# Autobot37/weatherforecastingtoolkit

Measured on AMD Instinct MI355X. Metric: SEVIR 384x384 frames/sec (AE train step), higher is better.
Workload: dtype f32; 1 GPU; experiments/ae_v2 conv AE (ae_64x8x8_lin.PosAwareAE_TF, img_size=384), 1x384x384 synthetic SEVIR frames, batch 32/GPU, fp32, fwd + L1 + bwd + AdamW + cosine-warmup LR; batch_per_gpu=32, global_batch=32, img_size=384, parallelism=dp1, params=215033281

## Files before the change

### include/wfae.h

```cpp
#ifndef WFAE_H
#define WFAE_H

#include <stddef.h>
#include <stdint.h>

#ifdef __cplusplus
extern "C" {
#endif

typedef void* wfae_stream_t;

typedef enum {
  WFAE_OK = 0,
  WFAE_ERR_BAD_SHAPE = -1,
  WFAE_ERR_NULL_POINTER = -2,
  WFAE_ERR_WORKSPACE = -3,
  WFAE_ERR_LAUNCH = -4,
  WFAE_ERR_UNSUPPORTED = -5
} wfae_status;

int wfae_version(void);
const char* wfae_last_error_string(void);
size_t wfae_workspace_bytes(int64_t max_weight_elems);

enum { WFAE_PRECISION_FP32 = 0, WFAE_PRECISION_BF16 = 1 };
int wfae_set_matmul_precision(int mode);
int wfae_get_matmul_precision(void);

int wfae_set_split_gemm(int on);
int wfae_get_split_gemm(void);

int wfae_set_c1n(int on);
int wfae_get_c1n(void);

int wfae_conv1x1_fwd(const float* x, const float* w, const float* bias, const float* res,
                     int64_t res_img_stride, float* y, int NB, int Cin, int Cout, int HW,
                     wfae_stream_t stream);
int wfae_conv1x1_fwd_stats(const float* x, const float* w, const float* bias, const float* res,
                           int64_t res_img_stride, float* y, int NB, int Cin, int Cout, int HW,
                           double* stat_part, int64_t stat_capacity, int* stat_rows, wfae_stream_t stream);
int wfae_conv1x1_fwd_bnact(const float* x, const float* bn_scale, const float* bn_shift, const float* w,
                           const float* bias, const float* res, int64_t res_img_stride, float* y, int NB, int Cin,
                           int Cout, int HW, double* stat_part, int64_t stat_capacity, int* stat_rows,
                           wfae_stream_t stream);
int wfae_conv1x1_bwd_weight_bnact(const float* dy, const float* x, const float* bn_scale, const float* bn_shift,
                                  float* dw, int NB, int Cin, int Cout, int HW, int accumulate, void* ws,
                                  size_t ws_bytes, wfae_stream_t stream);
int wfae_conv1x1_bwd_data(const float* dy, const float* w, float* dx, int NB, int Cin, int Cout,
                          int HW, wfae_stream_t stream);
int wfae_conv1x1_bwd_weight(const float* dy, const float* x, float* dw, int NB, int Cin, int Cout,
                            int HW, int accumulate, void* ws, size_t ws_bytes, wfae_stream_t stream);

int wfae_c1r_supported(int M, int K, int HW);
int wfae_c1r_stat_rows(int M, int K, int NB, int HW);
int wfae_c1r_fwd(const float* w, int64_t w_sm, int64_t w_sk, const float* x, const float* pro_scale, const float* pro_shift,
                 const float* res, float* y, int NB, int K, int M, int HW, double* stat_part, int64_t stat_capacity,
                 int* stat_rows, wfae_stream_t stream);
int wfae_c1r_bnred_supported(int M, int K, int HW);
int wfae_c1r_bnred(const float* w, int64_t w_sm, int64_t w_sk, const float* dt, const float* x, const float* bn_scale,
                   const float* bn_shift, const float* save_mean, const float* save_invstd, float* da, int NB, int K, int M, int HW,
                   double* part, int64_t part_capacity, int* part_rows, wfae_stream_t stream);
int wfae_bn_act_bwd_from_rows(const double* part, int rows, int C, float* dgamma, float* dbeta, int accumulate, void* ws,
                              size_t ws_bytes, wfae_stream_t stream);
int wfae_c1r_bndx(const float* w, int64_t w_sm, int64_t w_sk, const float* dt, const float* x, const float* gamma,
                  const float* bn_scale, const float* bn_shift, const float* save_mean, const float* save_invstd, const float* coef,
                  const float* res, float* dx, int NB, int K, int M, int HW, int training, wfae_stream_t stream);
int wfae_c1rb_supported(int M, int K, int HW);
int wfae_c1rb_stat_rows(int M, int K, int NB, int HW);
int wfae_c1rb_fwd(const float* w, int64_t w_sm, int64_t w_sk, const uint16_t* x, const float* pro_scale, const float* pro_shift,
                  const uint16_t* res, uint16_t* y, int NB, int K, int M, int HW, double* stat_part, int64_t stat_capacity,
                  int* stat_rows, wfae_stream_t stream);
int wfae_c1w_supported(int Cin, int Cout, int HW);
int wfae_c1w_bwd_weight(const float* dy, const float* x, const float* bn_scale, const float* bn_shift, float* dw, int NB, int Cin,
                        int Cout, int HW, int accumulate, void* ws, size_t ws_bytes, wfae_stream_t stream);
int wfae_c1w_bwd_weight_bf16(const uint16_t* dy, const uint16_t* x, const float* bn_scale, const float* bn_shift, float* dw, int NB,
                             int Cin, int Cout, int HW, int accumulate, void* ws, size_t ws_bytes, wfae_stream_t stream);
int wfae_set_c1wd(int on);
int wfae_get_c1wd(void);
int wfae_c1wd_supported(int C, int mid, int HW);
int wfae_c1wd_bwd(const float* dy, const float* t2, const float* bn_scale, const float* bn_shift, const float* w3, float* dw3,
                  float* da3, int NB, int C, int mid, int HW, int accumulate, void* ws, size_t ws_bytes, wfae_stream_t stream);
int wfae_linear_fwd(const float* x, const float* w, const float* bias, float* y, int B, int In,
                    int Out, void* ws, size_t ws_bytes, wfae_stream_t stream);
int wfae_linear_bwd_data(const float* dy, const float* w, float* dx, int B, int In, int Out,
                         wfae_stream_t stream);
int wfae_linear_bwd_weight(const float* dy, const float* x, float* dw, int B, int In, int Out,
                           int accumulate, wfae_stream_t stream);
int wfae_linear_bwd_data_splitk(const float* dy, const float* w, float* dx, int B, int In, int Out, void* ws,
                                size_t ws_bytes, wfae_stream_t stream);
int wfae_linear_bwd_weight_splitk(const float* dy, const float* x, float* dw, int B, int In, int Out, int accumulate,
                                  void* ws, size_t ws_bytes, wfae_stream_t stream);

int wfae_conv4x4s2_down(const float* hi, const float* w, float* lo, int NB, int Chi, int Clo,
                        int Hlo, int Wlo, wfae_stream_t stream);
int wfae_conv4x4s2_up(const float* lo, const float* w, float* hi, int NB, int Chi, int Clo, int Hlo,
                      int Wlo, void* ws, size_t ws_bytes, wfae_stream_t stream);
int wfae_conv4x4s2_wgrad(const float* lo, const float* hi, float* dw, int NB, int Chi, int Clo,
                         int Hlo, int Wlo, int accumulate, void* ws, size_t ws_bytes,
                         wfae_stream_t stream);

int wfae_dconv_fwd(const float* x, const float* w, const float* bias, float* y, int NB, int Cin,
                   int Cout, int H, int W, int KS, int stride, int pad, int groups,
                   wfae_stream_t stream);
int wfae_dconv_bwd_data(const float* dy, const float* w, float* dx, int NB, int Cin, int Cout,
                        int H, int W, int KS, int pad, int groups, wfae_stream_t stream);
int wfae_dconv_bwd_weight(const float* dy, const float* x, float* dw, int NB, int Cin, int Cout,
                          int H, int W, int KS, int stride, int pad, int groups, int accumulate,
                          void* ws, size_t ws_bytes, wfae_stream_t stream);

int wfae_gconv3x3_fwd(const float* x, const float* w, float* y, int NB, int C, int H, int W, int groups,
                      int transposed, void* ws, size_t ws_bytes, wfae_stream_t stream);
int wfae_gconv3x3_bwd_weight(const float* dy, const float* x, float* dw, int NB, int C, int H, int W,
                             int groups, int accumulate, void* ws, size_t ws_bytes, wfae_stream_t stream);

int wfae_bn_stats_train(const float* x, int NB, int C, int HW, const float* gamma,
                        const float* beta, float eps, float momentum, float* running_mean,
                        float* running_var, float* save_mean, float* save_invstd, float* scale,
                        float* shift, void* ws, size_t ws_bytes, wfae_stream_t stream);
int wfae_bn_stats_from_rows(const double* stat_part, int rows, int NB, int C, int HW, const float* gamma,
                            const float* beta, float eps, float momentum, float* running_mean,
                            float* running_var, float* save_mean, float* save_invstd, float* scale,
                            float* shift, void* ws, size_t ws_bytes, wfae_stream_t stream);
int wfae_bn_fold_eval(const float* gamma, const float* beta, const float* running_mean,
                      const float* running_var, float eps, float* save_mean, float* save_invstd,
                      float* scale, float* shift, int C, wfae_stream_t stream);
int wfae_bn_act_fwd(const float* x, const float* scale, const float* shift, float* y, int NB, int C,
                    int HW, int act, wfae_stream_t stream);
int wfae_bn_act_fwd_stats(const float* x, const float* scale, const float* shift, float* y, int NB, int C, int HW, int act,
                          double* part, int64_t part_capacity, int* splits_out, wfae_stream_t stream);
int wfae_bn_stats_from_parts(const double* part, int splits, int NB, int C, int HW, const float* gamma, const float* beta,
                             float eps, float momentum, float* running_mean, float* running_var, float* save_mean,
                             float* save_invstd, float* scale, float* shift, wfae_stream_t stream);
int wfae_bn_act_bwd(const float* dy, const float* x, const float* gamma, const float* scale,
                    const float* shift, const float* save_mean, const float* save_invstd,
                    const float* res, float* dx, float* dgamma, float* dbeta, int NB, int C, int HW,
                    int act, int training, int accumulate, int phases, void* ws, size_t ws_bytes,
                    wfae_stream_t stream);

int wfae_convert_f32_to_bf16(const float* src, uint16_t* dst, int64_t n, wfae_stream_t stream);
int wfae_convert_bf16_to_f32(const uint16_t* src, float* dst, int64_t n, wfae_stream_t stream);
int wfae_bn_stats_train_bf16(const uint16_t* x, int NB, int C, int HW, const float* gamma, const float* beta, float eps,
                             float momentum, float* running_mean, float* running_var, float* save_mean, float* save_invstd,
                             float* scale, float* shift, void* ws, size_t ws_bytes, wfae_stream_t stream);
int wfae_bn_act_fwd_bf16(const uint16_t* x, const float* scale, const float* shift, uint16_t* y, int NB, int C, int HW, int act,
                         wfae_stream_t stream);
int wfae_bn_act_fwd_stats_bf16(const uint16_t* x, const float* scale, const float* shift, uint16_t* y, int NB, int C, int HW,
                               int act, double* part, int64_t part_capacity, int* splits_out, wfae_stream_t stream);
int wfae_conv1x1_fwd_bf16(const uint16_t* x, const float* bn_scale, const float* bn_shift, const float* w, const float* bias,
                          const uint16_t* res, int64_t res_img_stride, uint16_t* y, int NB, int Cin, int Cout, int HW,
                          double* stat_part, int64_t stat_capacity, int* stat_rows, wfae_stream_t stream);
int wfae_conv1x1_bwd_data_bf16(const uint16_t* dy, const float* w, uint16_t* dx, int NB, int Cin, int Cout, int HW,
                               wfae_stream_t stream);
int wfae_conv1x1_bwd_weight_bf16(const uint16_t* dy, const uint16_t* x, const float* bn_scale, const float* bn_shift, float* dw,
                                 int NB, int Cin, int Cout, int HW, int accumulate, void* ws, size_t ws_bytes,
                                 wfae_stream_t stream);
int wfae_gconv3x3_fwd_bf16(const uint16_t* x, const float* w, uint16_t* y, int NB, int C, int H, int W, int groups,
                           int transposed, void* ws, size_t ws_bytes, wfae_stream_t stream);
int wfae_gconv3x3_bwd_weight_bf16(const uint16_t* dy, const uint16_t* x, float* dw, int NB, int C, int H, int W, int groups,
                                  int accumulate, void* ws, size_t ws_bytes, wfae_stream_t stream);
int wfae_dconv_fwd_bf16out(const float* x, const float* w, const float* bias, uint16_t* y, int NB, int Cout, int H, int W,
                           wfae_stream_t stream);
int wfae_dconv_fwd_bf16in(const uint16_t* x, const float* w, const float* bias, float* y, int NB, int Cin, int Cout, int H,
                          int W, wfae_stream_t stream);
int wfae_dconv_bwd_data_bf16out(const float* dy, const float* w, uint16_t* dx, int NB, int Cin, int H, int W,
// ... 316 lines not shown
```

### weatherforecastingtoolkit_amd/functional.py

```python
from __future__ import annotations

import os

import torch
from torch.autograd import Function

from . import ops

BN_EPS = 1e-5


_overlap = False
_side = {}


STAT_FUSION = os.environ.get("WFAE_STAT_FUSION", "1") == "1"


FUSE_A1 = os.environ.get("WFAE_FUSE_A1", "1") == "1"
FUSE_A1_MAXC = 1 << 30
FUSE_A3 = os.environ.get("WFAE_FUSE_A3", "1") == "1"
FUSE_A3_MAXC = int(os.environ.get("WFAE_FUSE_A3_MAXC", "128"))
FUSE_A3_MAXC_C1R = max(FUSE_A3_MAXC, 256)

# ... 374 lines not shown
        (x,) = ctx.saved_tensors
        return ops.leaky_relu_bwd(_c(dy), x)


class MeanFn(Function):

    @staticmethod
    def forward(ctx, x, hinge, sign, weight):
        x = _c(x)
        ctx.save_for_backward(x)
        ctx.cfg = (hinge, sign, weight)
        return ops.mean_fwd(x, hinge, sign, weight)

    @staticmethod
    def backward(ctx, g):
        (x,) = ctx.saved_tensors
        hinge, sign, weight = ctx.cfg
        return ops.mean_bwd(x, _c(g), hinge, sign, weight), None, None, None


class ScaleByFn(Function):

    @staticmethod
    def forward(ctx, x, s):
        ctx.save_for_backward(s)
        return ops.scale(_c(x), 1.0, s)

    @staticmethod
    def backward(ctx, g):
        (s,) = ctx.saved_tensors
        return ops.scale(_c(g), 1.0, s), None


def hinge_d_loss(logits_real, logits_fake):
    return AddFn.apply(MeanFn.apply(logits_real, True, -1.0, 0.5), MeanFn.apply(logits_fake, True, 1.0, 0.5))


def neg_mean(x):
    return MeanFn.apply(x, False, 1.0, -1.0)


def _g3_fwd(x, w, groups):
    if ops.gconv3x3_supported(x.shape[1], groups) and w.shape[0] == x.shape[1]:
        return ops.gconv3x3_fwd(x, w, groups, False)
    return ops.dconv_fwd(x, w, None, 3, 1, 1, groups)


def _g3_dgrad(dy, w, cin, groups):
    if ops.gconv3x3_supported(cin, groups) and w.shape[0] == cin:
        return ops.gconv3x3_fwd(dy, w, groups, True)
    return ops.dconv_bwd_data(dy, w, cin, 3, 1, groups)


def _g3_wgrad(dy, x, dw, groups):
    c = x.shape[1]
    if c % groups == 0 and c // groups in (4, 8, 16, 32) and dw.shape[0] == c and groups > 1:
        return ops.gconv3x3_bwd_weight(dy, x, dw, groups)
    return ops.dconv_bwd_weight(dy, x, dw, 3, 1, 1, groups)


def _mk_stats(mean, invstd, scale, shift):
    st = ops.BnStats.__new__(ops.BnStats)
    st.mean, st.invstd, st.scale, st.shift = mean, invstd, scale, shift
    return st


def _storage(t):
    return "bf16" if t.dtype == ops.BF16 else "f32"


def _c1(w, plane, transposed, x, st=None, res=None, stats=False, fam=None):
    if fam is None:
        fam = ops.conv1x1_route("dgrad" if transposed else "fwd", w.shape[1] if transposed else w.shape[0], x.shape[1],
                                x.shape[2] * x.shape[3], _storage(x), st is not None, False, "none" if res is None else "ordinary")
    if fam == "c1b" and (plane is None or plane.numel() == 0):
        fam = "gemm"
    label = None if fam in ("c1r", "gemm") else "wfae_c1b_dgrad" if transposed else "wfae_c1b_fwd"
    return ops._c1_launch(fam, plane if fam == "c1b" else w, transposed, x, st, None, res, False, stats, label)


_b16 = _c1


def _dgrad_bn(dt, w, Wt, x, gamma, st, dgamma, dbeta, res, training):
    how = ops.conv1x1_dgrad_bn_route(w.shape[1], dt.shape[1], dt.shape[2] * dt.shape[3], _storage(dt))
    if how is not None:
        da, sr = ops.c1r_bnred(w, dt, x, st, store=how == "bnred")
        ops.bn_act_bwd_from_rows(sr, x.shape[1], dgamma, dbeta)
        if how == "bndx":
            return ops.c1r_bndx(w, dt, x, gamma, st, res, training)
        return ops.bn_act_bwd_dx(da, x, gamma, st, res, 1, training)
    return ops.bn_act_bwd(_c1(w, Wt, True, dt)[0], x, gamma, st, dgamma, dbeta, res, 1, training)


class BottleneckFn(Function):
    @staticmethod
    def forward(ctx, x, g1, b1, w1, g2, b2, wg, g3, b3, w3, mod, x_stats=None):
        xc = _c(x)
        if xc is not x:
            x_stats = None
        x = xc
        bn1, bn2, bn3 = mod.f[0], mod.f[3], mod.f[6]
        groups = mod.f[5].groups
        training = _use_batch_stats(bn1)
        fuse = training and STAT_FUSION
        emit = fuse and getattr(mod, "emit_stats", False)
        C, mid, hw = x.shape[1], w1.shape[0], x.shape[2] * x.shape[3]
        sto = _storage(x)

        def route(op, m, k, pro=False, res="none"):
            return ops.conv1x1_route(op, m, k, hw, sto, pro, False, res)
        fused1 = FUSE_A1 and C <= FUSE_A1_MAXC and ops.conv1x1_bnact_supported(x, mid)
        r1, r3 = route("fwd", mid, C, fused1), route("fwd", C, mid, True, "ordinary")
        fused3 = (FUSE_A3 and C <= (FUSE_A3_MAXC_C1R if r3 in ("c1r", "c1rb") else FUSE_A3_MAXC)
                  and ops.conv1x1_bnact_supported((x.shape[0], mid) + x.shape[2:], C))
        if not fused3:
            r3 = route("fwd", C, mid, False, "ordinary")
        d1, d3 = (route("dgrad", C, mid), route("dgrad", mid, C)) if sto == "bf16" else (None, None)
        W1p, W3p = (ops.c1b_weights(w1), ops.c1b_weights(w3)) if "c1b" in (r1, r3, d1, d3) else ((None, None), (None, None))
        st1 = _bn_stats_rows(x_stats if (fuse or isinstance(x_stats, ops.StatParts)) else None, x, bn1, training)
        a1 = None if fused1 else ops.bn_act_fwd(x, st1, 1)
        t1, sr2 = _c1(w1, W1p[0], False, *((x, st1) if fused1 else (a1, None)), None, fuse, r1)
        st2 = _bn_stats_rows(sr2, t1, bn2, training)
        a2 = ops.bn_act_fwd(t1, st2, 1)
        t2 = _g3_fwd(a2, wg, groups)
        st3 = _bn_stats(t2, bn3, training)
        a3 = None if fused3 else ops.bn_act_fwd(t2, st3, 1)
        y, mod._out_stats = _c1(w3, W3p[0], False, *((t2, st3) if fused3 else (a3, None)), x, emit, r3)
        ctx.save_for_backward(x, _opt(a1), t1, a2, t2, _opt(a3), g1, w1, g2, wg, g3, w3,
                              st1.mean, st1.invstd, st1.scale, st1.shift,
                              st2.mean, st2.invstd, st2.scale, st2.shift,
                              st3.mean, st3.invstd, st3.scale, st3.shift,
                              _opt(W1p[1] if d1 == "c1b" else None), _opt(W3p[1] if d3 == "c1b" else None))
        ctx.training = training
        ctx.groups = groups
        ctx.betas = (b1, b2, b3)
        return y

    @staticmethod
    def backward(ctx, dy):
        (x, a1, t1, a2, t2, a3, g1, w1, g2, wg, g3, w3, *s) = ctx.saved_tensors
        st1, st2, st3 = _mk_stats(*s[0:4]), _mk_stats(*s[4:8]), _mk_stats(*s[8:12])
        W1t, W3t = s[12], s[13]
        tr = ctx.training
        dy = _c(dy)
        mid = w1.shape[0]
        dw3 = grad_buffer(w3)
        da3 = None
        if a3.numel() == 0:
            if ops.conv1x1_wd_route(dy.shape[1], mid, dy.shape[2] * dy.shape[3], _storage(dy)) == "c1wd":
                da3 = _on_main(lambda: ops.conv1x1_bwd_wd(dy, t2, st3, w3, dw3))
            if da3 is None:
                _wgrad(lambda: ops.conv1x1_bwd_weight_bnact(dy, t2, st3, dw3), dy, t2, st3.scale, st3.shift)
        else:
            _wgrad(lambda: ops.conv1x1_bwd_weight(dy, a3, dw3), dy, a3)
        dg3, db3 = grad_buffer(g3), grad_buffer(ctx.betas[2])
        if da3 is not None:
            dt2 = ops.bn_act_bwd(da3, t2, g3, st3, dg3, db3, None, 1, tr)
        else:
            dt2 = _dgrad_bn(dy, w3, W3t, t2, g3, st3, dg3, db3, None, tr)
        del da3
        dwg = grad_buffer(wg)
        _wgrad(lambda: _g3_wgrad(dt2, a2, dwg, ctx.groups), dt2, a2)
        da2 = _g3_dgrad(dt2, wg, mid, ctx.groups)
        del dt2
        dg2, db2 = grad_buffer(g2), grad_buffer(ctx.betas[1])
        dt1 = ops.bn_act_bwd(da2, t1, g2, st2, dg2, db2, None, 1, tr)
        del da2
        dw1 = grad_buffer(w1)
        if a1.numel() == 0:
            _wgrad(lambda: ops.conv1x1_bwd_weight_bnact(dt1, x, st1, dw1), dt1, x, st1.scale, st1.shift)
        else:
            _wgrad(lambda: ops.conv1x1_bwd_weight(dt1, a1, dw1), dt1, a1)
        dg1, db1 = grad_buffer(g1), grad_buffer(ctx.betas[0])
        dx = _dgrad_bn(dt1, w1, W1t, x, g1, st1, dg1, db1, dy, tr)
        return dx, dg1, db1, dw1, dg2, db2, dwg, dg3, db3, dw3, None, None


class Conv1x1Fn(Function):

    @staticmethod
    def forward(ctx, x, w, bias, pos):
        ctx.x_dtype = x.dtype
        x = ops.to_f32(_c(x))
        y = ops.conv1x1_fwd(x, w, bias, None if pos is None else _c(pos), pos is not None)
        ctx.save_for_backward(x, w)
        ctx.bias, ctx.pos = bias, pos
        return y

    @staticmethod
    def backward(ctx, dy):
        x, w = ctx.saved_tensors
        dy = ops.to_f32(_c(dy))
        nb, cout, h, wd = dy.shape
        dw = grad_buffer(w)
        ops.conv1x1_bwd_weight(dy, x, dw)
        dx = ops.to_dtype(ops.conv1x1_bwd_data(dy, w), ctx.x_dtype) if ctx.needs_input_grad[0] else None
        dbias = dpos = None
        if ctx.bias is not None:
            dbias = grad_buffer(ctx.bias)
            ops.reduce_sum(dy, nb, cout, h * wd, dbias)
        if ctx.pos is not None:
            dpos = grad_buffer(ctx.pos)
            ops.reduce_sum(dy, nb, cout * h * wd, 1, dpos)
        return dx, dw, dbias, dpos


def conv1x1(x, w, bias=None, pos=None):
    return Conv1x1Fn.apply(x, w, bias, pos)


class LinearFn(Function):
    @staticmethod
    def forward(ctx, x, w, bias):
        x = _c(x)
        y = ops.linear_fwd(x, w, bias)
        ctx.save_for_backward(x, w)
        ctx.bias = bias
        return y

    @staticmethod
    def backward(ctx, dy):
        x, w = ctx.saved_tensors
        dy = _c(dy)
        dw = grad_buffer(w)
        ops.linear_bwd_weight(dy, x, dw)
        dx = ops.linear_bwd_data(dy, w) if ctx.needs_input_grad[0] else None
        dbias = None
        if ctx.bias is not None:
            dbias = grad_buffer(ctx.bias)
            ops.reduce_sum(dy, dy.shape[0], w.shape[0], 1, dbias)
        return dx, dw, dbias


class DConvFn(Function):

    @staticmethod
    def forward(ctx, x, w, bias, groups):
        x = _c(x)
        y = ops.dconv_fwd(x, w, bias, 3, 1, 1, groups)
        ctx.save_for_backward(x, w)
        ctx.groups = groups
        ctx.bias = bias
        return y

    @staticmethod
    def backward(ctx, dy):
        x, w = ctx.saved_tensors
        dy = _c(dy)
        dw = grad_buffer(w)
        ops.dconv_bwd_weight(dy, x, dw, 3, 1, 1, ctx.groups)
        dx = ops.dconv_bwd_data(dy, w, x.shape[1], 3, 1, ctx.groups, out_dtype=x.dtype) if ctx.needs_input_grad[0] else None
        dbias = None
        if ctx.bias is not None:
            nb, cout, h, wd = dy.shape
            dbias = grad_buffer(ctx.bias)
            ops.reduce_sum(dy, nb, cout, h * wd, dbias)
        return dx, dw, dbias, None
# ... 982 lines not shown
```

### weatherforecastingtoolkit_amd/ops.py

```python
from __future__ import annotations

import ctypes
import os

import torch

from . import _lib

_WS_DEFAULT = int(os.environ.get("WFAE_WORKSPACE_MB", "512")) << 20
_ws = {}


def _stream():
    return torch.cuda.current_stream().cuda_stream


_prof = None


def profile_start():
    global _prof
    _prof = {}


# ... 128 lines not shown
    global _ACT_DTYPE
    if dtype not in (torch.float32, BF16):
        raise ValueError("activation storage is torch.float32 or torch.bfloat16")
    if dtype == BF16 and _lib.load().wfae_get_matmul_precision() != 1:
        raise _lib.WfaeError("bf16 activation storage needs set_float32_matmul_precision('medium')")
    _ACT_DTYPE = dtype


def to_f32(x):
    if x.dtype == torch.float32:
        return x
    _chka(x)
    y = torch.empty(x.shape, dtype=torch.float32, device=x.device)
    _call("wfae_convert_bf16_to_f32", 0, 6 * x.numel(), _p(x), _p(y), x.numel(), _stream())
    return y


def to_bf16(x):
    if x.dtype == BF16:
        return x
    _chk(x)
    y = torch.empty(x.shape, dtype=BF16, device=x.device)
    _call("wfae_convert_f32_to_bf16", 0, 6 * x.numel(), _p(x), _p(y), x.numel(), _stream())
    return y


def to_dtype(x, dtype):
    return to_bf16(x) if dtype == BF16 else to_f32(x)


def _p(t):
    return None if t is None else t.data_ptr()


class StatRows:
    __slots__ = ("part", "rows")

    def __init__(self, part, rows):
        self.part, self.rows = part, rows


class StatParts:
    __slots__ = ("part", "splits")

    def __init__(self, part, splits):
        self.part, self.splits = part, splits


def _rows_out(n, device):
    part = torch.empty(n, dtype=torch.float64, device=device)
    count = ctypes.c_int(0)
    return part, count, (part.data_ptr(), n, ctypes.cast(ctypes.pointer(count), ctypes.c_void_p))


_NO_ROWS = (None, 0, None)


_C1R = _C1R_BNRED = _C1R_BNDX = _C1RB = _C1B = _C1W = True


def set_c1r(on):
    global _C1R
    _C1R = bool(on)


def set_c1r_bnred(on):
    global _C1R_BNRED
    _C1R_BNRED = bool(on)


def set_c1r_bndx(on):
    global _C1R_BNDX
    _C1R_BNDX = bool(on)


def set_c1n(on):
    _lib.call("wfae_set_c1n", int(bool(on)))


def set_c1wd(on):
    _lib.call("wfae_set_c1wd", int(bool(on)))


def set_c1rb(on):
    global _C1RB
    _C1RB = bool(on)


def set_c1b(on):
    global _C1B
    _C1B = bool(on)


def set_c1w(on):
    global _C1W
    _C1W = bool(on)


def c1r_bndx_on():
    return _C1R_BNDX


def c1n_enabled():
    return bool(_lib.load().wfae_get_c1n())


def c1wd_enabled():
    return bool(_lib.load().wfae_get_c1wd())


def _precision():
    return _lib.load().wfae_get_matmul_precision()


def c1r_supported(m, k, hw):
    return _C1R and _SPLIT_GEMM and _precision() == 0 and bool(_lib.load().wfae_c1r_supported(int(m), int(k), int(hw)))


def c1r_bnred_supported(m, k, hw):
    return (_C1R and _C1R_BNRED and _SPLIT_GEMM and _precision() == 0
            and bool(_lib.load().wfae_c1r_bnred_supported(int(m), int(k), int(hw))))


def c1rb_supported(m, k, hw):
    return _C1RB and _precision() == 1 and bool(_lib.load().wfae_c1rb_supported(int(m), int(k), int(hw)))


def c1b_supported(m, k, hw):
    return _C1B and _precision() == 1 and bool(_lib.load().wfae_c1b_supported(int(m), int(k), int(hw)))


def conv1x1_bnact_supported(x, cout):
    nb, cin, h, wd = getattr(x, "shape", x)
    swapped = cin < cout and cin < 128
    return (h * wd) % 4 == 0 and h * wd >= 16 and cin % 4 == 0 and (cout % 4 == 0 or not swapped)


def conv1x1_route(op, m, k, hw, storage="f32", prologue=False, bias=False, residual="none"):
    if op == "wgrad":
        ok = _C1W and _lib.load().wfae_c1w_supported(int(k), int(m), int(hw))
        return "c1w" if ok and (_precision() == 1 if storage == "bf16" else (_precision() == 0 and _SPLIT_GEMM)) else "gemm"
    if bias or residual == "broadcast" or (residual == "ordinary" and m <= k):
        return "gemm"
    if storage == "f32":
        return "c1r" if c1r_supported(m, k, hw) else "gemm"
    rb = c1rb_supported(m, k, hw)
    if rb and not (prologue and m < k and k >= 256):
        return "c1rb"
    return "c1b" if (rb or c1b_supported(m, k, hw)) else "gemm"


def conv1x1_dgrad_bn_route(m, k, hw, storage="f32"):
    if storage == "f32" and c1r_bnred_supported(m, k, hw):
        return "bndx" if _C1R_BNDX else "bnred"
    return None


_C1_PEAK = {"c1r": PEAK_BF16_MFMA / 6, "c1rb": PEAK_BF16_MFMA, "c1b": PEAK_BF16_MFMA, "gemm": None}


def _c1_launch(fam, w, transposed, x, st=None, bias=None, res=None, res_broadcast=False, stats=False, label=None):
    sfx, es = _chka(x, res)
    nb, k, h, wd = x.shape
    hw, n = h * wd, nb * h * wd
    if fam == "c1b":
        if not sfx or w.dtype != BF16 or not w.is_contiguous() or w.shape[1] != k:
            raise _lib.WfaeError("c1b_fwd: bf16 activations and the contiguous (M, K) bf16 weight plane of c1b_weights")
        m = w.shape[0]
    else:
        _chk(w, bias)
        if fam != "gemm" and (fam == "c1rb") != bool(sfx):
            raise _lib.WfaeError(f"{fam}: {'bf16-stored' if fam == 'c1rb' else 'fp32'} activations")
        m = w.shape[1] if transposed else w.shape[0]
    y = torch.empty((nb, m, h, wd), dtype=x.dtype, device=x.device)
    by = es * n * (k + m) + w.element_size() * k * m + (0 if res is None else es * n * m)
    ps, ph = (None, None) if st is None else (_p(st.scale), _p(st.shift))
    label = label or ("wfae_conv1x1_bwd_data" if transposed else "wfae_conv1x1_fwd_bnact" if st is not None else "wfae_conv1x1_fwd")
    part, rows, out = None, None, _NO_ROWS
    if stats:
        cap = 4 * ((n + 127) // 128) * m if fam == "gemm" else 2 * int(getattr(_lib.load(), f"wfae_{fam}_stat_rows")(m, k, nb, hw)) * m
        part, rows, out = _rows_out(cap, x.device)
    if fam in ("c1r", "c1rb"):
        name, args = f"wfae_{fam}_fwd", (_p(w), *((1, m) if transposed else (k, 1)), _p(x), ps, ph, _p(res), _p(y), nb, k, m, hw, *out)
    elif fam == "c1b":
        name, args = "wfae_c1b_fwd", (_p(w), _p(x), ps, ph, _p(res), _p(y), nb, k, m, hw, *out)
    elif transposed:
        name, args = "wfae_conv1x1_bwd_data" + sfx, (_p(x), _p(w), _p(y), nb, m, k, hw)
    else:
        tail = (_p(w), _p(bias), _p(res), 0 if res_broadcast else m * hw, _p(y), nb, k, m, hw)
        if sfx or st is not None:
            name, args = "wfae_conv1x1_fwd" + (sfx or "_bnact"), (_p(x), ps, ph, *tail, *out)
# ... 48 lines not shown
    return _c1_launch(fam, w, True, dy)[0]


def c1rb_fwd(w, transposed, x, st=None, res=None, stats=False, label="wfae_c1b_fwd"):
    r = _c1_launch("c1rb", w, transposed, x, st, None, res, False, stats, label)
    return r if stats else r[0]


def c1b_weights(w):
    _chk(w)
    cout, cin = w.shape[0], w.shape[1]
    Wb = torch.empty((cout, cin), dtype=BF16, device=w.device)
    Wtb = torch.empty((cin, cout), dtype=BF16, device=w.device)
    _call("wfae_c1b_weights", 0, 8 * w.numel(), _p(w), _p(Wb), _p(Wtb), cout, cin, _stream())
    return Wb, Wtb


def c1b_fwd(Wb, x, st=None, res=None, stats=False, label="wfae_c1b_fwd"):
    r = _c1_launch("c1b", Wb, False, x, st, None, res, False, stats, label)
    return r if stats else r[0]


def _c1_wgrad(dy, x, st, dw, accumulate):
    sfx, es = _chka(dy, x)
    _chk(dw)
    nb, cout, h, wd = dy.shape
    cin, n = x.shape[1], nb * h * wd
    pro = (None, None) if st is None else (_p(st.scale), _p(st.shift))
    peak = None
    if conv1x1_route("wgrad", cout, cin, h * wd, "bf16" if sfx else "f32", st is not None) == "c1w":
        name, peak = "wfae_c1w_bwd_weight" + sfx, PEAK_BF16_MFMA / (1 if sfx else 6)
    elif sfx:
        name = "wfae_conv1x1_bwd_weight_bf16"
    else:
        name, pro = ("wfae_conv1x1_bwd_weight", ()) if st is None else ("wfae_conv1x1_bwd_weight_bnact", pro)
    ws = workspace()
    _call(name, 2 * n * cin * cout, es * n * (cin + cout) + 4 * cin * cout, _p(dy), _p(x), *pro, _p(dw), nb, cin, cout, h * wd,
          int(accumulate), ws.data_ptr(), ws.numel(), _stream(), peak=peak,
          label="wfae_conv1x1_bwd_weight" if st is None else "wfae_conv1x1_bwd_weight_bnact")
    return dw


def conv1x1_bwd_weight(dy, x, dw, accumulate=False):
    return _c1_wgrad(dy, x, None, dw, accumulate)


def conv1x1_bwd_weight_bnact(dy, x, st, dw, accumulate=False):
    return _c1_wgrad(dy, x, st, dw, accumulate)


C1WD_MIN_HW = 512


def conv1x1_wd_supported(c, mid, hw, storage="f32"):
    return (storage == "f32" and _SPLIT_GEMM and _precision() == 0 and bool(_lib.load().wfae_c1wd_supported(int(c), int(mid), int(hw)))
            and conv1x1_route("wgrad", c, mid, hw, "f32", True) == "c1w" and conv1x1_route("dgrad", mid, c, hw) == "c1r")


def conv1x1_wd_route(c, mid, hw, storage="f32"):
    return "c1wd" if hw >= C1WD_MIN_HW and conv1x1_wd_supported(c, mid, hw, storage) else "pair"


def conv1x1_bwd_wd(dy, t2, st, w3, dw3, accumulate=False):
    if st is None or dy.dtype != torch.float32 or t2.dtype != torch.float32:
        return None
    nb, c, h, wd = dy.shape
    mid, hw = t2.shape[1], h * wd
    if not conv1x1_wd_supported(c, mid, hw):
        return None
    _chk(dy, t2, w3, dw3)
    if tuple(t2.shape) != (nb, mid, h, wd) or w3.numel() != c * mid or dw3.numel() != c * mid:
        raise _lib.WfaeError("conv1x1_bwd_wd: dy (N, C, H, W), t2 (N, C/4, H, W), w3 and dw3 (C, C/4)")
    if (dy.data_ptr() | t2.data_ptr()) & 15:
        return None
    da = torch.empty_like(t2)
    n = nb * hw
    ws = workspace()
    _call("wfae_c1wd_bwd", 4 * n * c * mid, 4 * n * (c + 2 * mid) + 8 * c * mid, _p(dy), _p(t2), _p(st.scale), _p(st.shift), _p(w3),
          _p(dw3), _p(da), nb, c, mid, hw, int(accumulate), ws.data_ptr(), ws.numel(), _stream(), peak=PEAK_BF16_MFMA / 6,
          label="wfae_c1wd_bwd")
    return da


def c1r_bnred(w, dt, x, st, store=True):
    _chk(w, dt, x)
    nb, k, h, wd = dt.shape
    m, n = w.shape[1], nb * h * wd
    da = torch.empty((nb, m, h, wd), dtype=torch.float32, device=dt.device) if store else None
    part, rows, out = _rows_out(2 * int(_lib.load().wfae_c1r_stat_rows(m, k, nb, h * wd)) * m, dt.device)
    _call("wfae_c1r_bnred", 2 * n * k * m, 4 * (n * (k + (2 if store else 1) * m) + k * m), _p(w), 1, m, _p(dt), _p(x), _p(st.scale),
          _p(st.shift), _p(st.mean), _p(st.invstd), _p(da), nb, k, m, h * wd, *out, _stream(), label="wfae_conv1x1_bwd_data",
          peak=_C1_PEAK["c1r"])
    return da, StatRows(part[:2 * rows.value * m], rows.value)


def bn_act_bwd_from_rows(sr, c, dgamma, dbeta, accumulate=False):
    _chk(dgamma, dbeta)
    ws = workspace()
    _call("wfae_bn_act_bwd_from_rows", 0, 8 * sr.part.numel(), sr.part.data_ptr(), sr.rows, c, _p(dgamma), _p(dbeta), int(accumulate),
          ws.data_ptr(), ws.numel(), _stream(), label="wfae_bn_act_bwd[reduce]")
    return ws


def bn_act_bwd_dx(dy, x, gamma, st, res=None, act=1, training=True):
    _chk(dy, x, gamma, res)
    nb, c, h, wd = x.shape
    dx = torch.empty_like(x)
    ws = workspace()
    _call("wfae_bn_act_bwd", 0, 4 * x.numel() * (4 if res is not None else 3), _p(dy), _p(x), _p(gamma), _p(st.scale), _p(st.shift),
          _p(st.mean), _p(st.invstd), _p(res), _p(dx), None, None, nb, c, h * wd, act, int(training), 0, 2, ws.data_ptr(),
          ws.numel(), _stream(), label="wfae_bn_act_bwd[dx]")
    return dx


def c1r_bndx(w, dt, x, gamma, st, res=None, training=True):
    _chk(w, dt, x, gamma, res)
    nb, k, h, wd = dt.shape
    m, n = w.shape[1], nb * h * wd
    dx = torch.empty((nb, m, h, wd), dtype=torch.float32, device=dt.device)
    ws = workspace()
    _call("wfae_c1r_bndx", 2 * n * k * m, 4 * (n * (k + (3 if res is not None else 2) * m) + k * m), _p(w), 1, m, _p(dt), _p(x), _p(gamma),
          _p(st.scale), _p(st.shift), _p(st.mean), _p(st.invstd), ws.data_ptr(), _p(res), _p(dx), nb, k, m, h * wd, int(training),
          _stream(), label="wfae_c1r_bndx", peak=_C1_PEAK["c1r"])
    return dx


def linear_fwd(x, w, bias=None):
    _chk(x, w, bias)
    b, inf = x.shape
    out = w.shape[0]
    y = torch.empty((b, out), dtype=x.dtype, device=x.device)
    ws = workspace()
    _call("wfae_linear_fwd", 2 * b * inf * out, 4 * (inf * out + b * (inf + out)), _p(x), _p(w), _p(bias), _p(y), b, inf, out, ws.data_ptr(), ws.numel(), _stream())
    return y


def linear_bwd_data(dy, w):
    _chk(dy, w)
    b, out = dy.shape
    inf = w.shape[1]
    dx = torch.empty((b, inf), dtype=dy.dtype, device=dy.device)
    tiles = ((b + 127) // 128) * ((inf + 127) // 128)
    if tiles < 256 and out >= 512:
        ws = workspace(b * inf * 4 * 2)
        _call("wfae_linear_bwd_data_splitk", 2 * b * inf * out, 4 * (inf * out + b * (inf + out)), _p(dy), _p(w), _p(dx), b, inf,
              out, ws.data_ptr(), ws.numel(), _stream())
        return dx
    _call("wfae_linear_bwd_data", 2 * b * inf * out, 4 * (inf * out + b * (inf + out)), _p(dy), _p(w), _p(dx), b, inf, out, _stream())
    return dx


def linear_bwd_weight(dy, x, dw, accumulate=False):
    _chk(dy, x, dw)
    b, out = dy.shape
    inf = x.shape[1]
    tiles = ((out + 127) // 128) * ((inf + 127) // 128)
    if tiles < 256 and b >= 256:
        ws = workspace(out * inf * 4 * 2)
        _call("wfae_linear_bwd_weight_splitk", 2 * b * inf * out, 4 * (inf * out + b * (inf + out)), _p(dy), _p(x), _p(dw), b, inf,
              out, int(accumulate), ws.data_ptr(), ws.numel(), _stream())
        return dw
    _call("wfae_linear_bwd_weight", 2 * b * inf * out, 4 * (inf * out + b * (inf + out)), _p(dy), _p(x), _p(dw), b, inf, out, int(accumulate), _stream())
    return dw


_WINO_MODE = os.environ.get("WFAE_WINO", "auto")
# ... 1882 lines not shown
```

Baseline: 178.3 frames/s.

## Fuse bottleneck first-conv weight grad with BN-backward stat reduction

Adds a HIP kernel that, in one pass over x and dt1, computes the 1x1 conv weight gradient (split-bf16 MFMA on GELU(BN(x))) and the per-channel BN backward sums (recomputing da = W1^T dt1 on the fly). The bottleneck backward then uses these stat rows to skip the separate c1r_bnred dgrad-reduction pass and goes straight to the bndx kernel. This removes one full read of x and dt1 plus a GEMM launch. In exchange, the weight grad now runs on the main stream instead of the side wgrad stream, and the kernel does extra dgrad MFMA work.

Measured after the change: 181.8 frames/s (median of 6 runs). 1.02x the previous value.

```diff
diff --git a/include/wfae.h b/include/wfae.h
--- a/include/wfae.h
+++ b/include/wfae.h
@@ -80,6 +80,13 @@
 int wfae_c1wd_supported(int C, int mid, int HW);
 int wfae_c1wd_bwd(const float* dy, const float* t2, const float* bn_scale, const float* bn_shift, const float* w3, float* dw3,
                   float* da3, int NB, int C, int mid, int HW, int accumulate, void* ws, size_t ws_bytes, wfae_stream_t stream);
+int wfae_set_c1ws(int on);
+int wfae_get_c1ws(void);
+int wfae_c1ws_supported(int C, int mid, int HW);
+int wfae_c1ws_stat_rows(int C, int mid, int NB, int HW, size_t ws_bytes);
+int wfae_c1ws_bwd(const float* x, const float* dt1, const float* bn_scale, const float* bn_shift, const float* save_mean,
+                  const float* save_invstd, const float* w1, float* dw1, double* part, int64_t part_capacity, int* part_rows, int NB,
+                  int C, int mid, int HW, int accumulate, void* ws, size_t ws_bytes, wfae_stream_t stream);
 int wfae_linear_fwd(const float* x, const float* w, const float* bias, float* y, int B, int In,
                     int Out, void* ws, size_t ws_bytes, wfae_stream_t stream);
 int wfae_linear_bwd_data(const float* dy, const float* w, float* dx, int B, int In, int Out,
diff --git a/weatherforecastingtoolkit_amd/csrc/c1ws.hip b/weatherforecastingtoolkit_amd/csrc/c1ws.hip
--- /dev/null
+++ b/weatherforecastingtoolkit_amd/csrc/c1ws.hip
@@ -0,0 +1,397 @@
+#include "common.h"
+#include <atomic>
+#include <stdlib.h>
+#include <type_traits>
+
+using namespace wfae;
+
+namespace {
+
+typedef float f32x4 __attribute__((ext_vector_type(4)));
+typedef float f32x16 __attribute__((ext_vector_type(16)));
+typedef __bf16 bf16x8 __attribute__((ext_vector_type(8)));
+typedef short s16x4 __attribute__((ext_vector_type(4)));
+typedef unsigned u32x4 __attribute__((ext_vector_type(4)));
+typedef unsigned u32x2 __attribute__((ext_vector_type(2)));
+
+struct C1WSP {
+  const float* x;
+  const float* dt;
+  const float* w1;
+  const float* scale;
+  const float* shift;
+  const float* mean;
+  const float* invstd;
+  float* slab;
+  double* part0;
+  double* part1;
+  int HW;
+  int cpi;
+  int kc;
+};
+
+constexpr int SNT = 512, SBK = 32;
+constexpr int D_LD = 36;
+
+__device__ __forceinline__ unsigned off_row(int r, int c) { return (unsigned)(r * 64 + ((c ^ ((r >> 2) & 3)) << 4)); }
+
+__device__ __forceinline__ void split_pair(float a, float b, unsigned& h, unsigned& m, unsigned& l) {
+  h = pack_bf16(a, b);
+  const float ra = a - bf16_lo(h), rb = b - bf16_hi(h);
+  m = pack_bf16(ra, rb);
+  l = pack_bf16(ra - bf16_lo(m), rb - bf16_hi(m));
+}
+
+template <int C>
+__global__ __launch_bounds__(SNT, 2) void c1ws_kernel(C1WSP p) {
+  constexpr bool RCST = C == 128;
+  constexpr int M = C / 4;
+  constexpr int TM = C / 128;
+  constexpr int WQ = M / 32;
+  constexpr int NDW = 4 * WQ;
+  constexpr bool BOTH = NDW == 8;
+  constexpr int KCH = M / 32;
+  constexpr int RW = C / 8;
+  constexpr int RB = RW / 16;
+  constexpr int LPR = 8;
+  constexpr int P_IT = RW / 8;
+  constexpr int Q_LD = M * LPR;
+  static_assert(Q_LD <= SNT, "loader");
+  constexpr int A_PLANE_B = C * 64, B_PLANE_B = M * 64;
+  constexpr int A_STAGE_B = 3 * A_PLANE_B, STAGE_B = 3 * (A_PLANE_B + B_PLANE_B);
+  constexpr int D_WAVE_B = RW * D_LD * 4;
+  static_assert(2 * STAGE_B + 8 * D_WAVE_B <= 156 * 1024, "LDS");
+  __shared__ __attribute__((aligned(16))) unsigned char smem[2 * STAGE_B + 8 * D_WAVE_B];
+  const int t = threadIdx.x, lane = t & 63;
+  const int wave = __builtin_amdgcn_readfirstlane(t >> 6);
+  const int img = blockIdx.x / p.cpi, chunk = blockIdx.x - img * p.cpi;
+  const int k_begin = chunk * p.kc;
+  const int k_end = min(p.HW, k_begin + p.kc);
+  const int nsteps = (k_end - k_begin) / SBK;
+  const bool do_dw = BOTH || wave < NDW;
+
+  const int l_r = lane >> 3, l_e = lane & 7;
+  const int row0 = RW * wave;
+  const float* Pb = p.x + (long)img * C * p.HW + k_begin;
+  const float* Qb = p.dt + (long)img * M * p.HW + k_begin;
+  const float* p_src = Pb + (long)(row0 + l_r) * p.HW + l_e * 4;
+  const long p_step = 8l * p.HW;
+  const unsigned p_dst0 = off_row(row0 + l_r, l_e >> 1) + (unsigned)((l_e & 1) * 8);
+  auto p_dst = [&](int j) { return (p_dst0 ^ (unsigned)(32 * (j & 1))) + 512u * (unsigned)j; };
+  f32x4 rc[RCST ? P_IT : 1];
+  if constexpr (RCST) {
+#pragma unroll
+    for (int j = 0; j < P_IT; ++j) {
+      const int r = row0 + 8 * j + l_r;
+      rc[j] = f32x4{p.scale[r], p.shift[r], p.mean[r], p.invstd[r]};
+    }
+  } else {
+    const int r = row0 + (lane & (RW - 1));
+    rc[0] = f32x4{p.scale[r], p.shift[r], p.mean[r], p.invstd[r]};
+  }
+  const bool q_on = Q_LD == SNT || t < Q_LD;
+  const int q_r = q_on ? t / LPR : 0, q_e = t % LPR;
+  const float* q_src = Qb + (long)q_r * p.HW + q_e * 4;
+  const unsigned q_dst = off_row(q_r, q_e >> 1) + (unsigned)((q_e & 1) * 8);
+  u32x4 rp[P_IT], rq;
+  float gp[P_IT][4], xh[P_IT][4];
+  double sum1[P_IT], sum2[P_IT];
+#pragma unroll
+  for (int j = 0; j < P_IT; ++j) sum1[j] = sum2[j] = 0.0;
+  auto load_global = [&]() {
+#pragma unroll
+    for (int j = 0; j < P_IT; ++j) rp[j] = *reinterpret_cast<const u32x4*>(p_src + j * p_step);
+    if (q_on) rq = *reinterpret_cast<const u32x4*>(q_src);
+  };
+  auto advance = [&](bool more) {
+    p_src += more ? SBK : 0;
+    q_src += more ? SBK : 0;
+  };
+  auto put = [&](unsigned char* base, int plane_b, unsigned dst, float v0, float v1, float v2, float v3) {
+    unsigned h0, m0, l0, h1, m1, l1;
+    split_pair(v0, v1, h0, m0, l0);
+    split_pair(v2, v3, h1, m1, l1);
+    *reinterpret_cast<u32x2*>(base + dst) = u32x2{h0, h1};
+    *reinterpret_cast<u32x2*>(base + plane_b + dst) = u32x2{m0, m1};
+    *reinterpret_cast<u32x2*>(base + 2 * plane_b + dst) = u32x2{l0, l1};
+  };
+  auto store_lds = [&](int buf) {
+    unsigned char* s = smem + buf * STAGE_B;
+#pragma unroll
+    for (int j = 0; j < P_IT; ++j) {
+      const unsigned u0 = rp[j][0], u1 = rp[j][1], u2 = rp[j][2], u3 = rp[j][3];
+      const float x0 = __uint_as_float(u0), x1 = __uint_as_float(u1), x2 = __uint_as_float(u2), x3 = __uint_as_float(u3);
+      f32x4 cst;
+      if constexpr (RCST) cst = rc[j];
+      else {
+        const int from = 4 * (8 * j + l_r);
+#pragma unroll
+        for (int e = 0; e < 4; ++e) {
+          const float mine = rc[0][e];
+          cst[e] = __int_as_float(__builtin_amdgcn_ds_bpermute(from, __float_as_int(mine)));
+        }
+      }
+      const float a = cst.x, b = cst.y, mu = cst.z, is = cst.w;
+      const float w0 = fmaf(x0, a, b), w1 = fmaf(x1, a, b), w2 = fmaf(x2, a, b), w3 = fmaf(x3, a, b);
+      gp[j][0] = gelu_grad_f(w0); gp[j][1] = gelu_grad_f(w1); gp[j][2] = gelu_grad_f(w2); gp[j][3] = gelu_grad_f(w3);
+      xh[j][0] = (x0 - mu) * is; xh[j][1] = (x1 - mu) * is; xh[j][2] = (x2 - mu) * is; xh[j][3] = (x3 - mu) * is;
+      put(s, A_PLANE_B, p_dst(j), gelu_f(w0), gelu_f(w1), gelu_f(w2), gelu_f(w3));
+      if constexpr (!BOTH) __builtin_amdgcn_sched_barrier(0);
+    }
+    if (q_on) {
+      const unsigned u0 = rq[0], u1 = rq[1], u2 = rq[2], u3 = rq[3];
+      put(s + A_STAGE_B, B_PLANE_B, q_dst, __uint_as_float(u0), __uint_as_float(u1), __uint_as_float(u2), __uint_as_float(u3));
+    }
+  };
+
+  const int wm0 = (BOTH ? (wave >> 1) : (wave & 3)) * (32 * TM), wn0 = BOTH ? (wave & 1) * 32 : 0;
+  const int r31 = lane & 31, lh = lane >> 5;
+  const unsigned a_rd = (unsigned)((wm0 + r31) * 64), b_rd = (unsigned)((wn0 + r31) * 64);
+  const int a_x = (r31 >> 2) & 3;
+  f32x16 acc[TM];
+  struct Frag {
+    bf16x8 a[TM][3], b[3];
+  };
+  auto read_frag = [&](Frag& f, int buf, int ks) {
+    const unsigned char* s = smem + buf * STAGE_B;
+    const unsigned a_c = (unsigned)(((2 * ks + lh) ^ a_x) << 4);
+#pragma unroll
+    for (int i = 0; i < TM; ++i)
+#pragma unroll
+      for (int pl = 0; pl < 3; ++pl)
+        f.a[i][pl] = *reinterpret_cast<const bf16x8*>(s + pl * A_PLANE_B + a_rd + i * (32 * 64) + a_c);
+#pragma unroll
+    for (int pl = 0; pl < 3; ++pl) f.b[pl] = *reinterpret_cast<const bf16x8*>(s + A_STAGE_B + pl * B_PLANE_B + b_rd + a_c);
+  };
+  auto mfma_frag = [&](const Frag& f) {
+#pragma unroll
+    for (int i = 0; i < TM; ++i) {
+      f32x16 c = acc[i];
+      c = __builtin_amdgcn_mfma_f32_32x32x16_bf16(f.a[i][2], f.b[0], c, 0, 0, 0);
+      c = __builtin_amdgcn_mfma_f32_32x32x16_bf16(f.a[i][0], f.b[2], c, 0, 0, 0);
+      c = __builtin_amdgcn_mfma_f32_32x32x16_bf16(f.a[i][1], f.b[1], c, 0, 0, 0);
+      c = __builtin_amdgcn_mfma_f32_32x32x16_bf16(f.a[i][1], f.b[0], c, 0, 0, 0);
+      c = __builtin_amdgcn_mfma_f32_32x32x16_bf16(f.a[i][0], f.b[1], c, 0, 0, 0);
+      c = __builtin_amdgcn_mfma_f32_32x32x16_bf16(f.a[i][0], f.b[0], c, 0, 0, 0);
+      acc[i] = c;
+    }
+  };
+
+  const int n16 = lane & 15, kg = lane >> 4, tq = n16 >> 2, tp = n16 & 3;
+  bf16x8 wa[RB][KCH][3];
+#pragma unroll
+  for (int rb = 0; rb < RB; ++rb)
+#pragma unroll
+    for (int ch = 0; ch < KCH; ++ch) {
+      const float* src = p.w1 + (long)(32 * ch + 8 * kg) * C + row0 + 16 * rb + n16;
+      float v[8];
+#pragma unroll
+      for (int e = 0; e < 8; ++e) v[e] = src[e * C];
+      u32x4 h, m, l;
+#pragma unroll
+      for (int e = 0; e < 4; ++e) {
+        unsigned qh, qm, ql;
+        split_pair(v[2 * e], v[2 * e + 1], qh, qm, ql);
+        h[e] = qh; m[e] = qm; l[e] = ql;
+      }
+      wa[rb][ch][0] = __builtin_bit_cast(bf16x8, h);
+      wa[rb][ch][1] = __builtin_bit_cast(bf16x8, m);
+      wa[rb][ch][2] = __builtin_bit_cast(bf16x8, l);
+    }
+  __builtin_amdgcn_sched_barrier(0);
+  const unsigned tr_rd0 = off_row(8 * kg + tq, tp >> 1) + 8u * (unsigned)(tp & 1);
+  auto tr_rd = [&](int pt, int hf) { return (tr_rd0 ^ (unsigned)(16 * hf + 32 * pt)) + 256u * (unsigned)hf; };
+  unsigned char* const dtile = smem + 2 * STAGE_B + wave * D_WAVE_B;
+  float* const d_wr = reinterpret_cast<float*>(dtile) + (4 * kg) * D_LD + n16;
+  const unsigned char* const d_rd = dtile + (l_r * D_LD + 4 * l_e) * 4;
+  auto da_step = [&](int buf) {
+    const unsigned char* s = smem + buf * STAGE_B + A_STAGE_B;
+    constexpr int PA[6] = {2, 0, 1, 1, 0, 0}, PB[6] = {0, 2, 1, 0, 1, 0};
+#pragma unroll
+    for (int pt = 0; pt < 2; ++pt) {
+      bf16x8 b[KCH][3];
+#pragma unroll
+      for (int ch = 0; ch < KCH; ++ch)
+#pragma unroll
+        for (int pl = 0; pl < 3; ++pl) {
+          s16x4 part[2];
+#pragma unroll
+          for (int hf = 0; hf < 2; ++hf)
+            part[hf] = __builtin_amdgcn_ds_read_tr16_b64_v4i16(
+                (s16x4 __attribute__((address_space(3)))*)(s + pl * B_PLANE_B + ch * (32 * 64) + tr_rd(pt, hf)));
+          b[ch][pl] = __builtin_bit_cast(bf16x8, __builtin_shufflevector(part[0], part[1], 0, 1, 2, 3, 4, 5, 6, 7));
+        }
+#pragma unroll
+      for (int rb = 0; rb < RB; ++rb) {
+        f32x4 d = {0.f, 0.f, 0.f, 0.f};
+#pragma unroll
+        for (int ch = 0; ch < KCH; ++ch)
+#pragma unroll
+          for (int pr = 0; pr < 6; ++pr) d = __builtin_amdgcn_mfma_f32_16x16x32_bf16(wa[rb][ch][PA[pr]], b[ch][PB[pr]], d, 0, 0, 0);
+#pragma unroll
+        for (int q = 0; q < 4; ++q) d_wr[(16 * rb + q) * D_LD + 16 * pt] = d[q];
+      }
+    }
+  };
+  auto sums_step = [&]() {
+    __builtin_amdgcn_fence(__ATOMIC_RELEASE, "wavefront");
+    __builtin_amdgcn_wave_barrier();
+    __builtin_amdgcn_fence(__ATOMIC_ACQUIRE, "wavefront");
+#pragma unroll
+    for (int j = 0; j < P_IT; ++j) {
+      const f32x4 v = *reinterpret_cast<const f32x4*>(d_rd + j * (8 * D_LD * 4));
+      const float d0 = v.x * gp[j][0], d1 = v.y * gp[j][1];
+      const float d2 = v.z * gp[j][2], d3 = v.w * gp[j][3];
+      const float h0 = xh[j][0], h1 = xh[j][1], h2 = xh[j][2], h3 = xh[j][3];
+      const float s1 = (d0 + d1) + (d2 + d3);
+      const float s2 = fmaf(d0, h0, d1 * h1) + fmaf(d2, h2, d3 * h3);
+      sum1[j] += (double)s1;
+      sum2[j] += (double)s2;
+    }
+    __builtin_amdgcn_fence(__ATOMIC_RELEASE, "wavefront");
+    __builtin_amdgcn_wave_barrier();
+  };
+
+  auto run = [&](auto dwc) {
+    constexpr bool DW = decltype(dwc)::value;
+    if constexpr (DW) {
+#pragma unroll
+      for (int i = 0; i < TM; ++i)
+#pragma unroll
+        for (int q = 0; q < 16; ++q) acc[i][q] = 0.f;
+    }
+    if (nsteps > 0) {
+      Frag f0, f1;
+      load_global();
+      advance(nsteps > 1);
+      store_lds(0);
+      load_global();
+      advance(nsteps > 2);
+      __syncthreads();
+      for (int st = 0; st < nsteps; ++st) {
+        const int cur = st & 1;
+        da_step(cur);
+        sums_step();
+        __builtin_amdgcn_sched_barrier(0);
+        if (st + 1 < nsteps) store_lds(cur ^ 1);
+        load_global();
+        advance(st + 3 < nsteps);
+        __builtin_amdgcn_sched_barrier(0);
+        if constexpr (DW && BOTH) {
+          read_frag(f0, cur, 0);
+          read_frag(f1, cur, 1);
+          mfma_frag(f0);
+          mfma_frag(f1);
+        } else if constexpr (DW) {
+          read_frag(f0, cur, 0);
+          mfma_frag(f0);
+          read_frag(f0, cur, 1);
+          mfma_frag(f0);
+        }
+        __builtin_amdgcn_sched_barrier(0);
+        __syncthreads();
+        __builtin_amdgcn_sched_barrier(0);
+      }
+    }
+    if constexpr (DW) {
+      float* __restrict__ Cb = p.slab + (long)blockIdx.x * C * M;
+#pragma unroll
+      for (int i = 0; i < TM; ++i)
+#pragma unroll
+        for (int q = 0; q < 16; ++q) {
+          const int row = wm0 + 32 * i + (q & 3) + 8 * (q >> 2) + 4 * lh;
+          Cb[(long)row * M + wn0 + r31] = acc[i][q];
+        }
+    }
+  };
+  if constexpr (BOTH) run(std::true_type{});
+  else if (do_dw) run(std::true_type{});
+  else run(std::false_type{});
+
+#pragma unroll
+  for (int j = 0; j < P_IT; ++j) {
+    double e1 = sum1[j], e2 = sum2[j];
+#pragma unroll
+    for (int o = 1; o < 8; o <<= 1) {
+      e1 += __shfl_xor(e1, o, 64);
+      e2 += __shfl_xor(e2, o, 64);
+    }
+    if (l_e == 0) {
+      const long at = (long)blockIdx.x * C + row0 + 8 * j + l_r;
+      p.part0[at] = e1;
+      p.part1[at] = e2;
+    }
+  }
+}
+
+std::atomic<int> g_c1ws{-1};
+inline bool c1ws_on() {
+  int v = g_c1ws.load(std::memory_order_relaxed);
+  if (v < 0) {
+    const char* e = getenv("WFAE_C1WS");
+    v = (e && e[0] == '0') ? 0 : 1;
+    g_c1ws.store(v, std::memory_order_relaxed);
+  }
+  return v == 1;
+}
+
+inline bool al16(const void* q) { return (reinterpret_cast<uintptr_t>(q) & 15) == 0; }
+
+inline bool c1ws_shape_ok(int C, int mid, int HW) { return (C == 128 || C == 256) && mid * 4 == C && HW > 0 && HW % 64 == 0; }
+
+}
+
+extern "C" {
+
+int wfae_set_c1ws(int on) {
+  g_c1ws.store(on ? 1 : 0, std::memory_order_relaxed);
+  return WFAE_OK;
+}
+
+int wfae_get_c1ws(void) { return c1ws_on() ? 1 : 0; }
+
+int wfae_c1ws_supported(int C, int mid, int HW) {
+  return (c1ws_on() && c1ws_shape_ok(C, mid, HW) && wfae::split_gemm_enabled()) ? 1 : 0;
+}
+
+int wfae_c1ws_stat_rows(int C, int mid, int NB, int HW, size_t ws_bytes) {
+  int cpi = 0, kc = 0;
+  if (!c1ws_shape_ok(C, mid, HW) || NB <= 0 || !c1w_chunks(C, mid, NB, HW, ws_bytes, &cpi, &kc)) return 0;
+  return NB * cpi;
+}
+
+int wfae_c1ws_bwd(const float* x, const float* dt1, const float* bn_scale, const float* bn_shift, const float* save_mean,
+                  const float* save_invstd, const float* w1, float* dw1, double* part, int64_t part_capacity, int* part_rows, int NB,
+                  int C, int mid, int HW, int accumulate, void* ws, size_t ws_bytes, wfae_stream_t stream) {
+  WFAE_REQUIRE(x && dt1 && bn_scale && bn_shift && save_mean && save_invstd && w1 && dw1 && part && part_rows && ws,
+               WFAE_ERR_NULL_POINTER, "c1ws_bwd: null pointer");
+  WFAE_REQUIRE(NB > 0 && C > 0 && mid > 0 && HW > 0 && NB <= 65535 && (int64_t)NB * HW < (1ll << 31), WFAE_ERR_BAD_SHAPE,
+               "c1ws_bwd: bad shape");
+  WFAE_REQUIRE(c1ws_shape_ok(C, mid, HW), WFAE_ERR_UNSUPPORTED,
+               "c1ws_bwd: serves C = 128 or 256 with mid = C / 4 and HW %% 64 == 0 (C %d, mid %d, HW %d)", C, mid, HW);
+  WFAE_REQUIRE(c1ws_on() && wfae::split_gemm_enabled(), WFAE_ERR_UNSUPPORTED,
+               "c1ws_bwd: needs fp32 precision with the split GEMMs on and wfae_set_c1ws(1)");
+  WFAE_REQUIRE(al16(x) && al16(dt1), WFAE_ERR_UNSUPPORTED, "c1ws_bwd: x and dt1 must be 16-byte aligned");
+  C1WSP p = {};
+  p.x = x; p.dt = dt1; p.w1 = w1;
+  p.scale = bn_scale; p.shift = bn_shift; p.mean = save_mean; p.invstd = save_invstd;
+  p.slab = (float*)ws;
+  p.HW = HW;
+  WFAE_REQUIRE(c1w_chunks(C, mid, NB, HW, ws_bytes, &p.cpi, &p.kc), WFAE_ERR_WORKSPACE, "c1ws_bwd: workspace %zu < %zu", ws_bytes,
+               (size_t)NB * C * mid * sizeof(float));
+  const int rows = NB * p.cpi;
+  WFAE_REQUIRE(part_capacity >= 2 * (int64_t)rows * C, WFAE_ERR_WORKSPACE, "c1ws_bwd: part holds %lld doubles, needs %lld",
+               (long long)part_capacity, (long long)(2 * (int64_t)rows * C));
+  *part_rows = rows;
+  p.part0 = part;
+  p.part1 = part + (long)rows * C;
+  hipStream_t st = (hipStream_t)stream;
+  const dim3 grid((unsigned)rows), block(SNT);
+  if (C == 128) hipLaunchKernelGGL((c1ws_kernel<128>), grid, block, 0, st, p);
+  else hipLaunchKernelGGL((c1ws_kernel<256>), grid, block, 0, st, p);
+  const int rc = check_launch("c1ws_bwd");
+  if (rc) return rc;
+  return slab_reduce((const float*)ws, dw1, nullptr, (long)C * mid, mid, rows, accumulate, st, C);
+}
+
+}
diff --git a/weatherforecastingtoolkit_amd/functional.py b/weatherforecastingtoolkit_amd/functional.py
--- a/weatherforecastingtoolkit_amd/functional.py
+++ b/weatherforecastingtoolkit_amd/functional.py
@@ -480,7 +480,10 @@
 _b16 = _c1
 
 
-def _dgrad_bn(dt, w, Wt, x, gamma, st, dgamma, dbeta, res, training):
+def _dgrad_bn(dt, w, Wt, x, gamma, st, dgamma, dbeta, res, training, rows=None):
+    if rows is not None:
+        ops.bn_act_bwd_from_rows(rows, x.shape[1], dgamma, dbeta)
+        return ops.c1r_bndx(w, dt, x, gamma, st, res, training)
     how = ops.conv1x1_dgrad_bn_route(w.shape[1], dt.shape[1], dt.shape[2] * dt.shape[3], _storage(dt))
     if how is not None:
         da, sr = ops.c1r_bnred(w, dt, x, st, store=how == "bnred")
@@ -566,12 +569,16 @@
         dt1 = ops.bn_act_bwd(da2, t1, g2, st2, dg2, db2, None, 1, tr)
         del da2
         dw1 = grad_buffer(w1)
+        rows1 = None
         if a1.numel() == 0:
-            _wgrad(lambda: ops.conv1x1_bwd_weight_bnact(dt1, x, st1, dw1), dt1, x, st1.scale, st1.shift)
+            if ops.conv1x1_ws_route(x.shape[1], mid, x.shape[2] * x.shape[3], _storage(x)) == "c1ws":
+                rows1 = _on_main(lambda: ops.conv1x1_bwd_ws(dt1, x, st1, w1, dw1))
+            if rows1 is None:
+                _wgrad(lambda: ops.conv1x1_bwd_weight_bnact(dt1, x, st1, dw1), dt1, x, st1.scale, st1.shift)
         else:
             _wgrad(lambda: ops.conv1x1_bwd_weight(dt1, a1, dw1), dt1, a1)
         dg1, db1 = grad_buffer(g1), grad_buffer(ctx.betas[0])
-        dx = _dgrad_bn(dt1, w1, W1t, x, g1, st1, dg1, db1, dy, tr)
+        dx = _dgrad_bn(dt1, w1, W1t, x, g1, st1, dg1, db1, dy, tr, rows1)
         return dx, dg1, db1, dw1, dg2, db2, dwg, dg3, db3, dw3, None, None
 
 
diff --git a/weatherforecastingtoolkit_amd/ops.py b/weatherforecastingtoolkit_amd/ops.py
--- a/weatherforecastingtoolkit_amd/ops.py
+++ b/weatherforecastingtoolkit_amd/ops.py
@@ -234,6 +234,10 @@
     _lib.call("wfae_set_c1wd", int(bool(on)))
 
 
+def set_c1ws(on):
+    _lib.call("wfae_set_c1ws", int(bool(on)))
+
+
 def set_c1rb(on):
     global _C1RB
     _C1RB = bool(on)
@@ -259,6 +263,10 @@
 
 def c1wd_enabled():
     return bool(_lib.load().wfae_get_c1wd())
+
+
+def c1ws_enabled():
+    return bool(_lib.load().wfae_get_c1ws())
 
 
 def _precision():
@@ -473,6 +481,39 @@
     return da
 
 
+def conv1x1_ws_supported(c, mid, hw, storage="f32"):
+    return (storage == "f32" and _SPLIT_GEMM and _precision() == 0 and bool(_lib.load().wfae_c1ws_supported(int(c), int(mid), int(hw)))
+            and conv1x1_route("wgrad", mid, c, hw, "f32", True) == "c1w" and conv1x1_dgrad_bn_route(c, mid, hw, storage) == "bndx")
+
+
+def conv1x1_ws_route(c, mid, hw, storage="f32"):
+    return "c1ws" if hw >= C1WD_MIN_HW and conv1x1_ws_supported(c, mid, hw, storage) else "pair"
+
+
+def conv1x1_bwd_ws(dt1, x, st, w1, dw1, accumulate=False):
+    if st is None or dt1.dtype != torch.float32 or x.dtype != torch.float32:
+        return None
+    nb, c, h, wd = x.shape
+    mid, hw = dt1.shape[1], h * wd
+    if not conv1x1_ws_supported(c, mid, hw):
+        return None
+    _chk(dt1, x, w1, dw1)
+    if tuple(dt1.shape) != (nb, mid, h, wd) or w1.numel() != c * mid or dw1.numel() != c * mid:
+        raise _lib.WfaeError("conv1x1_bwd_ws: x (N, C, H, W), dt1 (N, C/4, H, W), w1 and dw1 (C/4, C)")
+    if (dt1.data_ptr() | x.data_ptr()) & 15:
+        return None
+    n = nb * hw
+    ws = workspace()
+    cap = 2 * int(_lib.load().wfae_c1ws_stat_rows(c, mid, nb, hw, ws.numel())) * c
+    if cap <= 0:
+        return None
+    part, rows, out = _rows_out(cap, x.device)
+    _call("wfae_c1ws_bwd", 4 * n * c * mid, 4 * n * (c + mid) + 8 * c * mid, _p(x), _p(dt1), _p(st.scale), _p(st.shift), _p(st.mean),
+          _p(st.invstd), _p(w1), _p(dw1), *out, nb, c, mid, hw, int(accumulate), ws.data_ptr(), ws.numel(), _stream(),
+          peak=PEAK_BF16_MFMA / 6, label="wfae_c1ws_bwd")
+    return StatRows(part[:2 * rows.value * c], rows.value)
+
+
 def c1r_bnred(w, dt, x, st, store=True):
     _chk(w, dt, x)
     nb, k, h, wd = dt.shape
```
